# giolucasd/ssrl-vit-mae-jepa

Hardware: AMD Instinct MI355X
Metric: images/sec pretrain step (fwd+bwd+opt), ViT-S/8 96px MAE, 1/2/4/8 MI355X (higher is better)
Workload: dtype bf16; 1 GPU; ViT-S/8 96px MAE (enc 384x12x6h, dec 192x2x6h, mask_ratio 0.75), batch 2000/GPU, full step; global_batch=2000, per_gpu_batch=2000, parallelism=dp1

## Files before the change

ssrl_vit_mae_jepa_amd/csrc/engine.hip:

```cpp
#include <string>
#include <vector>
#include <cmath>
#include <cstring>
#include <cstdlib>
#include <cstdint>
#include "kernels.h"

namespace mae {

static thread_local char g_err[1024] = "";
void set_error(const char* fmt, ...) {
  va_list ap;
  va_start(ap, fmt);
  vsnprintf(g_err, sizeof(g_err), fmt, ap);
  va_end(ap);
}
int hip_fail(hipError_t err, const char* what, const char* file, int line) {
  set_error("HIP error %d (%s) at %s:%d: %s", (int)err, hipGetErrorString(err), file, line, what);
  return 2;
}

struct ParamInfo {
  std::string name;
  int64_t offset = 0, numel = 0;
// ... 21 lines not shown

using namespace mae;

struct mae_engine {
  mae_config_t cfg;
  int act = MAE_F32;
  int D, depth, H, Dd, dd, Hd, P, L, G, C, img, p, mlp;
  int PO;
  std::vector<ParamInfo> params;
  int64_t arena_elems = 0, trainable_elems = 0, trans_elems = 0;
  int i_enc_mask, i_cls, i_pos, i_patch_w, i_patch_b, i_norm_w, i_norm_b;
  int i_dec_mask, i_dec_pos, i_de_w, i_de_b, i_dn_w, i_dn_b, i_pred_w, i_pred_b;
  std::vector<BlockRefs> enc, dec;
  bool timers_on = false;
  TimerSlot timers[TK_COUNT];
  int side_mode = -1;
  hipStream_t side = nullptr;
  std::vector<hipEvent_t> ev_pool;
  size_t ev_used = 0;
  PartialsTable ln_tab;
  hipEvent_t pending[4] = {nullptr, nullptr, nullptr, nullptr};
};

namespace mae {

static int add_param(mae_engine* e, const std::string& name, std::initializer_list<int64_t> shape, int flags) {
  ParamInfo pi;
  pi.name = name;
  pi.ndim = (int)shape.size();
  pi.numel = 1;
  int i = 0;
  for (int64_t s : shape) { pi.shape[i++] = s; pi.numel *= s; }
  pi.flags = flags;
  e->params.push_back(pi);
  return (int)e->params.size() - 1;
}
// ... 18 lines not shown

struct LayerBufs {
  int64_t x_mid, ln1, mean1, rstd1, qkv, lse, att, ln2, mean2, rstd2, fc1_pre, fc1_act;
};

struct Plan {
  int B, k, m;
  int dec_B, dec_T;
  int64_t Me, Md, Mp;
  int64_t keep32, mask32, inv, pred_rows;
  int64_t patchA;
  std::vector<int64_t> enc_x, dec_x;
  std::vector<LayerBufs> enc, dec;
  int64_t enc_norm, enc_mean, enc_rstd, xdec, dec_norm, dec_mean, dec_rstd, pred;
  int64_t branch_a, branch_b;
  int64_t dpred, d_decn, dres, dres_c, d_ln, d_att, d_qkv, d_hidden, d_xdec, dtok;
  int64_t ln_partial, ln_partial_stride, split_partial, wgrad_scratch, loss_scratch;
  int64_t total;
};

static Plan make_plan_ex(const mae_engine* e, int B, int k, int dec_B, int dec_T, int m_seq) {
  Plan pl;
  pl.B = B; pl.k = k; pl.m = m_seq;
  pl.dec_B = dec_B; pl.dec_T = dec_T;
  pl.Me = (int64_t)B * k; pl.Md = (int64_t)dec_B * dec_T; pl.Mp = (int64_t)dec_B * m_seq;
  const int64_t as = (int64_t)dtype_size(e->act);
  int64_t off = 0;
  auto take = [&](int64_t bytes) { const int64_t o = off; off += round_up(std::max<int64_t>(bytes, 4), 256); return o; };
  pl.keep32 = take(pl.Me * 4);
  pl.mask32 = take(pl.Mp * 4);
  pl.inv = take(pl.Md * 4);
// ... 19 lines not shown
  };
  layers(e->depth, pl.Me, e->D, e->H, k, pl.enc_x, pl.enc);
  pl.enc_norm = take(pl.Me * e->D * as); pl.enc_mean = take(pl.Me * 4); pl.enc_rstd = take(pl.Me * 4);
  pl.xdec = take(pl.Me * e->Dd * as);
  layers(e->dd, pl.Md, e->Dd, e->Hd, dec_T, pl.dec_x, pl.dec);
  pl.dec_norm = take(std::max<int64_t>(pl.Mp, 1) * e->Dd * as);
  pl.dec_mean = take(std::max<int64_t>(pl.Mp, 1) * 4); pl.dec_rstd = take(std::max<int64_t>(pl.Mp, 1) * 4);
  pl.pred = take(std::max<int64_t>(pl.Mp, 1) * e->PO * 4);
  const int64_t R = std::max(pl.Me * e->D, pl.Md * e->Dd);
  pl.branch_a = take(R * as);
  pl.branch_b = take(R * as);
  pl.dpred = take(std::max<int64_t>(pl.Mp, 1) * e->PO * as);
  pl.d_decn = take(std::max<int64_t>(pl.Mp, 1) * e->Dd * as);
  pl.dres = take(R * 4);
  pl.dres_c = take(R * as);
  pl.d_ln = take(R * as);
  pl.d_att = take(R * as);
  pl.d_qkv = take(3 * R * as);
  pl.d_hidden = take((int64_t)e->mlp * R * as);
  pl.d_xdec = take(pl.Me * e->Dd * as);
  pl.dtok = take(pl.Me * e->D * as);
  const int maxd = std::max(e->D, e->Dd);
  pl.ln_partial_stride = (int64_t)2 * LN_BWD_MAX_BLOCKS * maxd * 4;
  pl.ln_partial = take(pl.ln_partial_stride * std::min(2 * (e->depth + e->dd) + 2, (int)PartialsTable::MAX));
  pl.split_partial = take((int64_t)512 * maxd * 4);
  int64_t wg = 0;
  auto wgs = [&](int64_t M, int N, int K) { wg = std::max(wg, linear_wgrad_scratch_bytes(M, N, K)); };
  wgs(pl.Me, 3 * e->D, e->D); wgs(pl.Me, e->mlp * e->D, e->D); wgs(pl.Me, e->D, e->mlp * e->D); wgs(pl.Me, e->D, e->D);
  wgs(pl.Md, 3 * e->Dd, e->Dd); wgs(pl.Md, e->mlp * e->Dd, e->Dd); wgs(pl.Md, e->Dd, e->mlp * e->Dd); wgs(pl.Md, e->Dd, e->Dd);
  wgs(pl.Me, e->D, e->P); wgs(pl.Me, e->Dd, e->D); wgs(std::max<int64_t>(pl.Mp, 1), e->PO, e->Dd);
// ... 22 lines not shown
    (void)hipEventRecord(t.ev[t.used].first, s);
    stop = t.ev[t.used].second;
    t.used++;
    t.flops += flops;
    t.bytes += bytes;
  }
  ~TimerScope() { if (stop) (void)hipEventRecord(stop, s); }
};

#define RUN(kind, flops, bytes, expr)                      \
  do {                                                     \
    TimerScope _ts(e, kind, (double)(flops), (double)(bytes), s); \
    MAE_TRY(expr);                                         \
  } while (0)

enum DepTag { DEP_DRESC = 0, DEP_HIDDEN = 1, DEP_QKV = 2, DEP_MISC = 3 };

static bool side_enabled(mae_engine* e) {
  if (e->side_mode < 0) {
    const char* v = getenv("MAE_WGRAD_STREAM");
    e->side_mode = (v && v[0] == '1') ? 1 : 0;
    if (e->side_mode == 1 && hipStreamCreateWithFlags(&e->side, hipStreamNonBlocking) != hipSuccess) e->side_mode = 0;
  }
  return e->side_mode == 1;
}
static hipEvent_t next_event(mae_engine* e) {
  if (e->ev_used == e->ev_pool.size()) {
    hipEvent_t ev;
    if (hipEventCreateWithFlags(&ev, hipEventDisableTiming) != hipSuccess) return nullptr;
    e->ev_pool.push_back(ev);
  }
  return e->ev_pool[e->ev_used++];
}
static int await_side(mae_engine* e, int tag, hipStream_t s) {
  if (e->pending[tag]) {
    MAE_HIP(hipStreamWaitEvent(s, e->pending[tag], 0));
    e->pending[tag] = nullptr;
  }
  return 0;
// ... 33 lines not shown
  RUN(TK_LINEAR, 2.0 * M * N * K, gemm_bytes(M, N, K, c.as, (int64_t)dtype_size(out_dt), mode), launch_linear_fwd(A, c.W(wi), M, N, K, c.act, ep, s));
  return 0;
}

static int dgrad(const Ctx& c, const void* dY, int wi, int64_t M, int N, int K, int mode, void* out, const void* aux) {
  mae_engine* e = c.e; hipStream_t s = c.s;
  Epi ep; ep.mode = mode; ep.aux = aux; ep.out = out; ep.out_dt = c.act;
  if (c.act == MAE_BF16) {
    RUN(TK_LINEAR, 2.0 * M * N * K, gemm_bytes(M, K, N, 2, 2, mode), launch_linear_fwd(dY, c.WT(wi), M, K, N, MAE_BF16, ep, s));
  } else {
    RUN(TK_LINEAR, 2.0 * M * N * K, gemm_bytes(M, K, N, 4, 4, mode), launch_linear_dgrad(dY, c.W(wi), M, N, K, MAE_F32, ep, s));
  }
  return 0;
}

static int wgrad(const Ctx& c, const Plan& pl, const void* dY, const void* A, int64_t M, int N, int K, int wi, int bi, int tag) {
  mae_engine* e = c.e;
  hipStream_t s = c.s;
  const bool side = side_enabled(e);
  if (side) {
    hipEvent_t ready = next_event(e);
    MAE_REQUIRE(ready, "wgrad: cannot create an event");
    MAE_HIP(hipEventRecord(ready, c.s));
    MAE_HIP(hipStreamWaitEvent(e->side, ready, 0));
    s = e->side;
  }
  RUN(TK_WGRAD, 2.0 * M * N * K, (double)(M * (N + K) * c.as + (int64_t)N * K * 4),
      launch_linear_wgrad(dY, A, M, N, K, c.act, c.Gp(wi), bi >= 0 ? c.Gp(bi) : nullptr, c.buf<>(pl.wgrad_scratch), s));
  if (side) {
    hipEvent_t done = next_event(e);
    MAE_REQUIRE(done, "wgrad: cannot create an event");
    MAE_HIP(hipEventRecord(done, e->side));
    e->pending[tag] = done;
  }
  return 0;
}

static int wgrad_pair(const Ctx& c, const Plan& pl, int64_t M, const void* dY0, const void* A0, int N0, int K0, int w0, int b0,
                      const void* dY1, const void* A1, int N1, int K1, int w1, int b1) {
  mae_engine* e = c.e;
  hipStream_t s = c.s;
  RUN(TK_WGRAD, 2.0 * M * ((double)N0 * K0 + (double)N1 * K1),
      (double)(M * (int64_t)(N0 + K0 + N1 + K1) * c.as + ((int64_t)N0 * K0 + (int64_t)N1 * K1) * 4),
      launch_linear_wgrad_pair(dY0, A0, N0, K0, c.Gp(w0), c.Gp(b0), dY1, A1, N1, K1, c.Gp(w1), c.Gp(b1), M, c.act, c.buf<>(pl.wgrad_scratch), s));
  return 0;
}

static int join_side(const Ctx& c) {
  mae_engine* e = c.e;
  if (e->side_mode == 1) {
    hipEvent_t done = next_event(e);
    MAE_REQUIRE(done, "cannot create an event");
    MAE_HIP(hipEventRecord(done, e->side));
    MAE_HIP(hipStreamWaitEvent(c.s, done, 0));
    for (auto& p : e->pending) p = nullptr;
  }
  return 0;
}

static int block_forward(const Ctx& c, const Plan& pl, const BlockRefs& r, const LayerBufs& b, int64_t M, int d, int heads, int Bn, int T,
                         int64_t x_prev, bool add_prev, int64_t x_in) {
  mae_engine* e = c.e; hipStream_t s = c.s;
  const int hd = d / heads, hid = e->mlp * d;
  const float eps = 1e-6f;
  if (add_prev) {
// ... 9 lines not shown
    MAE_TRY(linear(c, c.buf<>(b.ln2), r.fc1_w, r.fc1_b, M, hid, d, MAE_EPI_GELU_ACT, c.act, c.buf<>(b.fc1_act), nullptr, nullptr));
  else
    MAE_TRY(linear(c, c.buf<>(b.ln2), r.fc1_w, r.fc1_b, M, hid, d, MAE_EPI_GELU_GRAD, c.act, c.buf<>(b.fc1_pre), c.buf<>(b.fc1_act), nullptr));
  MAE_TRY(linear(c, c.buf<>(b.fc1_act), r.fc2_w, r.fc2_b, M, d, hid, MAE_EPI_NONE, c.act, c.buf<>(pl.branch_b), nullptr, nullptr));
  return 0;
}

static float* ln_slot(const Ctx& c, const Plan& pl) { return c.buf<float>(pl.ln_partial + (int64_t)(c.e->ln_tab.n % PartialsTable::MAX) * pl.ln_partial_stride); }

static int block_backward(const Ctx& c, const Plan& pl, const BlockRefs& r, const LayerBufs& b, int64_t M, int d, int heads, int Bn, int T,
                          int64_t x_in) {
  mae_engine* e = c.e; hipStream_t s = c.s;
  const int hd = d / heads, hid = e->mlp * d;
  float* dres = c.buf<float>(pl.dres);
  void* dres_c = c.buf<>(pl.dres_c);
  if (!side_enabled(e)) {
    MAE_TRY(dgrad(c, dres_c, r.fc2_w, M, d, hid, MAE_EPI_MUL, c.buf<>(pl.d_hidden), c.buf<>(b.fc1_pre)));
    MAE_TRY(wgrad_pair(c, pl, M, dres_c, c.buf<>(b.fc1_act), d, hid, r.fc2_w, r.fc2_b, c.buf<>(pl.d_hidden), c.buf<>(b.ln2), hid, d, r.fc1_w, r.fc1_b));
    MAE_TRY(dgrad(c, c.buf<>(pl.d_hidden), r.fc1_w, M, hid, d, MAE_EPI_NONE, c.buf<>(pl.d_ln), nullptr));
    RUN(TK_LN_BWD, 0, M * d * (12 + 2 * c.as), launch_layernorm_bwd(c.buf<>(pl.d_ln), c.act, c.buf<float>(b.x_mid), nullptr, c.P(r.ln2_w), c.buf<float>(b.mean2), c.buf<float>(b.rstd2), M, d, 1, dres, dres_c, c.Gp(r.ln2_w), c.Gp(r.ln2_b), ln_slot(c, pl), s, &e->ln_tab));
    MAE_TRY(dgrad(c, dres_c, r.proj_w, M, d, d, MAE_EPI_NONE, c.buf<>(pl.d_att), nullptr));
    RUN(TK_ATTN_BWD, 10.0 * Bn * heads * (double)T * T * hd, M * 9 * d * c.as, launch_attention_bwd(c.buf<>(b.qkv), c.buf<>(b.att), c.buf<>(pl.d_att), c.buf<float>(b.lse), Bn, T, heads, hd, c.act, c.buf<>(pl.d_qkv), s));
    MAE_TRY(wgrad_pair(c, pl, M, dres_c, c.buf<>(b.att), d, d, r.proj_w, r.proj_b, c.buf<>(pl.d_qkv), c.buf<>(b.ln1), 3 * d, d, r.qkv_w, r.qkv_b));
    MAE_TRY(dgrad(c, c.buf<>(pl.d_qkv), r.qkv_w, M, 3 * d, d, MAE_EPI_NONE, c.buf<>(pl.d_ln), nullptr));
    RUN(TK_LN_BWD, 0, M * d * (12 + 2 * c.as), launch_layernorm_bwd(c.buf<>(pl.d_ln), c.act, c.buf<float>(x_in), nullptr, c.P(r.ln1_w), c.buf<float>(b.mean1), c.buf<float>(b.rstd1), M, d, 1, dres, dres_c, c.Gp(r.ln1_w), c.Gp(r.ln1_b), ln_slot(c, pl), s, &e->ln_tab));
    return 0;
  }
  MAE_TRY(wgrad(c, pl, dres_c, c.buf<>(b.fc1_act), M, d, hid, r.fc2_w, r.fc2_b, DEP_DRESC));
  MAE_TRY(await_side(e, DEP_HIDDEN, s));
  MAE_TRY(dgrad(c, dres_c, r.fc2_w, M, d, hid, MAE_EPI_MUL, c.buf<>(pl.d_hidden), c.buf<>(b.fc1_pre)));
  MAE_TRY(wgrad(c, pl, c.buf<>(pl.d_hidden), c.buf<>(b.ln2), M, hid, d, r.fc1_w, r.fc1_b, DEP_HIDDEN));
  MAE_TRY(dgrad(c, c.buf<>(pl.d_hidden), r.fc1_w, M, hid, d, MAE_EPI_NONE, c.buf<>(pl.d_ln), nullptr));
  MAE_TRY(await_side(e, DEP_DRESC, s));
  RUN(TK_LN_BWD, 0, M * d * (12 + 2 * c.as), launch_layernorm_bwd(c.buf<>(pl.d_ln), c.act, c.buf<float>(b.x_mid), nullptr, c.P(r.ln2_w), c.buf<float>(b.mean2), c.buf<float>(b.rstd2), M, d, 1, dres, dres_c, c.Gp(r.ln2_w), c.Gp(r.ln2_b), ln_slot(c, pl), s, &e->ln_tab));
  MAE_TRY(wgrad(c, pl, dres_c, c.buf<>(b.att), M, d, d, r.proj_w, r.proj_b, DEP_DRESC));
  MAE_TRY(dgrad(c, dres_c, r.proj_w, M, d, d, MAE_EPI_NONE, c.buf<>(pl.d_att), nullptr));
  MAE_TRY(await_side(e, DEP_QKV, s));
  RUN(TK_ATTN_BWD, 10.0 * Bn * heads * (double)T * T * hd, M * 9 * d * c.as, launch_attention_bwd(c.buf<>(b.qkv), c.buf<>(b.att), c.buf<>(pl.d_att), c.buf<float>(b.lse), Bn, T, heads, hd, c.act, c.buf<>(pl.d_qkv), s));
  MAE_TRY(wgrad(c, pl, c.buf<>(pl.d_qkv), c.buf<>(b.ln1), M, 3 * d, d, r.qkv_w, r.qkv_b, DEP_QKV));
  MAE_TRY(dgrad(c, c.buf<>(pl.d_qkv), r.qkv_w, M, 3 * d, d, MAE_EPI_NONE, c.buf<>(pl.d_ln), nullptr));
  MAE_TRY(await_side(e, DEP_DRESC, s));
  RUN(TK_LN_BWD, 0, M * d * (12 + 2 * c.as), launch_layernorm_bwd(c.buf<>(pl.d_ln), c.act, c.buf<float>(x_in), nullptr, c.P(r.ln1_w), c.buf<float>(b.mean1), c.buf<float>(b.rstd1), M, d, 1, dres, dres_c, c.Gp(r.ln1_w), c.Gp(r.ln1_b), ln_slot(c, pl), s, &e->ln_tab));
  return 0;
}

static int check_call(const mae_engine* e, const void* params, const void* wcache, int B, int k, const void* ws, int64_t ws_bytes,
                      Plan* pl, const char* who) {
  MAE_REQUIRE(e, "%s: null engine", who);
  MAE_REQUIRE(params && ws, "%s: null params/workspace", who);
  MAE_REQUIRE(e->act == MAE_F32 || wcache, "%s: bf16 engine needs the weight cache", who);
  MAE_REQUIRE(B > 0 && k >= 1 && k <= e->L, "%s: batch %d / num_keep %d out of range (L = %d)", who, B, k, e->L);
  MAE_REQUIRE((int64_t)B * e->L * std::max(3 * e->D, e->mlp * std::max(e->D, e->Dd)) < (1ll << 40), "%s: batch too large", who);
  *pl = make_plan(e, B, k);
  MAE_REQUIRE(ws_bytes >= pl->total, "%s: workspace too small (%lld < %lld bytes)", who, (long long)ws_bytes, (long long)pl->total);
  MAE_REQUIRE(((uintptr_t)ws & 255) == 0 && ((uintptr_t)params & 15) == 0, "%s: workspace must be 256-byte aligned, params 16-byte", who);
  return 0;
// ... 49 lines not shown
  return 0;
}

static int reach_point(const Ctx& c, int j) {
  mae_engine* e = c.e; hipStream_t s = c.s;
  if (!c.ready || !c.ready[j]) return 0;
  if (e->ln_tab.n > 0) {
    RUN(TK_LN_BWD, 0, 0, launch_sum_partials_many(e->ln_tab, s));
    e->ln_tab.n = 0;
  }
  MAE_TRY(join_side(c));
  MAE_HIP(hipEventRecord((hipEvent_t)c.ready[j], s));
  return 0;
}

static void backward_begin(const Ctx& c) {
  mae_engine* e = c.e;
  e->ev_used = 0;
  for (auto& p : e->pending) p = nullptr;
  e->ln_tab.n = 0;
}
static int backward_end(const Ctx& c) {
  mae_engine* e = c.e; hipStream_t s = c.s;
  if (e->ln_tab.n > 0) RUN(TK_LN_BWD, 0, 0, launch_sum_partials_many(e->ln_tab, s));
  e->ln_tab.n = 0;
  return join_side(c);
}

static int backward_decoder_impl(const Ctx& c, const Plan& pl, const JepaSeq* jp = nullptr) {
  mae_engine* e = c.e; hipStream_t s = c.s;
  float* dres = c.buf<float>(pl.dres);
  void* dres_c = c.buf<>(pl.dres_c);
  MAE_TRY(wgrad(c, pl, c.buf<>(pl.dpred), c.buf<>(pl.dec_norm), pl.Mp, e->PO, e->Dd, e->i_pred_w, e->i_pred_b, DEP_MISC));
  MAE_TRY(dgrad(c, c.buf<>(pl.dpred), e->i_pred_w, pl.Mp, e->PO, e->Dd, MAE_EPI_NONE, c.buf<>(pl.d_decn), nullptr));
  MAE_TRY(await_side(e, DEP_DRESC, s));
// ... 15 lines not shown
  float* dres = c.buf<float>(pl.dres);
  void* dres_c = c.buf<>(pl.dres_c);
  MAE_TRY(await_side(e, DEP_DRESC, s));
  RUN(TK_LN_BWD, 0, pl.Me * e->D * (12 + 2 * c.as), launch_layernorm_bwd(c.buf<>(pl.d_ln), c.act, c.buf<float>(pl.enc_x[e->depth]), nullptr, c.P(e->i_norm_w), c.buf<float>(pl.enc_mean), c.buf<float>(pl.enc_rstd), pl.Me, e->D, 0, dres, dres_c, c.Gp(e->i_norm_w), c.Gp(e->i_norm_b), ln_slot(c, pl), s, &e->ln_tab));
  for (int i = e->depth - 1; i >= 0; --i) {
    MAE_TRY(block_backward(c, pl, e->enc[i], pl.enc[i], pl.Me, e->D, e->H, pl.B, pl.k, pl.enc_x[i]));
    if (i > 0) MAE_TRY(reach_point(c, e->depth - i));
  }
  RUN(TK_DATA, 0, pl.Me * e->D * (4 + c.as), launch_visible_grad_split(dres, c.buf<int32_t>(pl.keep32), pl.Me, e->D, c.act, c.buf<>(pl.dtok), c.Gp(e->i_cls), c.buf<float>(pl.split_partial), s));
  MAE_TRY(wgrad(c, pl, c.buf<>(pl.dtok), c.buf<>(pl.patchA), pl.Me, e->D, e->P, e->i_patch_w, e->i_patch_b, DEP_MISC));
  return 0;
}

static int backward_impl(const Ctx& c, const Plan& pl, const float* d_x_encoded_extra = nullptr, const JepaSeq* jp = nullptr) {
  mae_engine* e = c.e; hipStream_t s = c.s;
  backward_begin(c);
  MAE_TRY(backward_decoder_impl(c, pl, jp));
  if (d_x_encoded_extra) MAE_TRY(launch_add_into(d_x_encoded_extra, c.buf<>(pl.d_ln), c.act, pl.Me * e->D, s));
  MAE_TRY(backward_encoder_impl(c, pl));
  MAE_TRY(backward_end(c));
  if (c.ready && c.ready[e->depth]) MAE_HIP(hipEventRecord((hipEvent_t)c.ready[e->depth], s));
  return 0;
}

}

extern "C" const char* mae_last_error(void) { return mae::g_err; }
extern "C" int mae_abi_version(void) { return MAE_ABI_VERSION; }

extern "C" int mae_engine_create(const mae_config_t* cfg, mae_engine_t** out) {
  MAE_REQUIRE(cfg && out, "mae_engine_create: null argument");
// ... 10 lines not shown
  for (int hd : {cfg->embed_dim / cfg->num_heads, cfg->decoder_embed_dim / cfg->decoder_num_heads})
    MAE_REQUIRE(hd == 16 || hd == 24 || hd == 32 || hd == 48 || hd == 64,
                "head dim %d is not supported by the attention kernels (16, 24, 32, 48 or 64): choose num_heads accordingly", hd);
  const int P = cfg->patch_size * cfg->patch_size * cfg->in_chans;
  MAE_REQUIRE(P % 4 == 0, "patch_size^2 * in_chans must be a multiple of 4");
  MAE_REQUIRE(cfg->pred_dim >= 0 && cfg->pred_dim % 4 == 0, "pred_dim must be 0 (pixels) or a multiple of 4");
  mae_engine* e = new mae_engine();
  e->cfg = *cfg;
  e->act = cfg->act_dtype;
  e->D = cfg->embed_dim; e->depth = cfg->depth; e->H = cfg->num_heads;
  e->Dd = cfg->decoder_embed_dim; e->dd = cfg->decoder_depth; e->Hd = cfg->decoder_num_heads;
  e->C = cfg->in_chans; e->img = cfg->image_size; e->p = cfg->patch_size;
  e->G = e->img / e->p; e->L = e->G * e->G + 1; e->P = P;
  e->mlp = cfg->mlp_ratio > 0 ? cfg->mlp_ratio : 4;
  e->PO = cfg->pred_dim > 0 ? cfg->pred_dim : P;
  const int T = MAE_PARAM_TRAINABLE, M = MAE_PARAM_TRAINABLE | MAE_PARAM_MATRIX;
  e->i_enc_mask = add_param(e, "encoder.mask_token", {1, 1, e->D}, MAE_PARAM_UNUSED);
  e->i_cls = add_param(e, "encoder.vit.cls_token", {1, 1, e->D}, T);
  e->i_pos = add_param(e, "encoder.vit.pos_embed", {1, e->L, e->D}, MAE_PARAM_FROZEN);
  e->i_patch_w = add_param(e, "encoder.vit.patch_embed.proj.weight", {e->D, e->C, e->p, e->p}, M);
  e->i_patch_b = add_param(e, "encoder.vit.patch_embed.proj.bias", {e->D}, T);
  for (int i = 0; i < e->depth; ++i) e->enc.push_back(add_block(e, "encoder.vit.blocks." + std::to_string(i), e->D, e->mlp));
  e->i_norm_w = add_param(e, "encoder.vit.norm.weight", {e->D}, T);
  e->i_norm_b = add_param(e, "encoder.vit.norm.bias", {e->D}, T);
  e->i_dec_mask = add_param(e, "decoder.mask_token", {1, 1, e->Dd}, T);
  e->i_dec_pos = add_param(e, "decoder.decoder_pos_embed", {1, e->L, e->Dd}, MAE_PARAM_FROZEN);
  e->i_de_w = add_param(e, "decoder.decoder_embed.weight", {e->Dd, e->D}, M);
  e->i_de_b = add_param(e, "decoder.decoder_embed.bias", {e->Dd}, T);
  for (int i = 0; i < e->dd; ++i) e->dec.push_back(add_block(e, "decoder.decoder_blocks." + std::to_string(i), e->Dd, e->mlp));
  e->i_dn_w = add_param(e, "decoder.decoder_norm.weight", {e->Dd}, T);
// ... 121 lines not shown
  Ctx c{e, params, (const char*)wcache, grads, (char*)workspace, s, e->act, (int64_t)dtype_size(e->act)};
  MAE_TRY(launch_cast(d_pred, MAE_F32, c.buf<>(pl.dpred), e->act, pl.Mp * e->PO, s));
  return backward_impl(c, pl, d_x_encoded_extra);
}

extern "C" int mae_engine_backward_decoder(mae_engine_t* e, const float* params, const void* wcache, const float* d_pred,
                                           int32_t batch, int32_t num_keep, int32_t num_mask, void* workspace,
                                           int64_t workspace_bytes, float* grads, float* d_x_encoded, void* stream) {
  Plan pl;
  MAE_TRY(check_call(e, params, wcache, batch, num_keep, workspace, workspace_bytes, &pl, "mae_engine_backward_decoder"));
  MAE_REQUIRE(d_pred && grads, "mae_engine_backward_decoder: null d_pred/grads");
  MAE_REQUIRE(num_mask == pl.m && pl.m > 0, "mae_engine_backward_decoder: num_mask mismatch");
  hipStream_t s = (hipStream_t)stream;
  Ctx c{e, params, (const char*)wcache, grads, (char*)workspace, s, e->act, (int64_t)dtype_size(e->act)};
  MAE_TRY(launch_cast(d_pred, MAE_F32, c.buf<>(pl.dpred), e->act, pl.Mp * e->PO, s));
  backward_begin(c);
  MAE_TRY(backward_decoder_impl(c, pl));
  MAE_TRY(backward_end(c));
  if (d_x_encoded) MAE_TRY(launch_cast(c.buf<>(pl.d_ln), e->act, d_x_encoded, MAE_F32, pl.Me * e->D, s));
  return 0;
}

extern "C" int mae_engine_backward_encoder(mae_engine_t* e, const float* params, const void* wcache, const float* d_x_encoded,
                                           int32_t batch, int32_t num_keep, void* workspace, int64_t workspace_bytes,
                                           float* grads, void* stream) {
  Plan pl;
  MAE_TRY(check_call(e, params, wcache, batch, num_keep, workspace, workspace_bytes, &pl, "mae_engine_backward_encoder"));
  MAE_REQUIRE(d_x_encoded && grads, "mae_engine_backward_encoder: null d_x_encoded/grads");
  hipStream_t s = (hipStream_t)stream;
  Ctx c{e, params, (const char*)wcache, grads, (char*)workspace, s, e->act, (int64_t)dtype_size(e->act)};
  MAE_TRY(launch_cast(d_x_encoded, MAE_F32, c.buf<>(pl.d_ln), e->act, pl.Me * e->D, s));
  backward_begin(c);
  MAE_TRY(backward_encoder_impl(c, pl));
  return backward_end(c);
}

extern "C" int64_t mae_engine_encoder_grad_elems(const mae_engine_t* e) { return e ? e->params[e->i_dec_mask].offset : 0; }

extern "C" int mae_engine_decoder_decode(mae_engine_t* e, const float* params, const void* wcache, const float* x, int32_t batch,
                                         void* workspace, int64_t workspace_bytes, float* out, void* stream) {
  Plan pl;
  MAE_TRY(check_call(e, params, wcache, batch, 1, workspace, workspace_bytes, &pl, "mae_engine_decoder_decode"));
  MAE_REQUIRE(x && out, "mae_engine_decoder_decode: null x/out");
  hipStream_t s = (hipStream_t)stream;
  Ctx c{e, params, (const char*)wcache, nullptr, (char*)workspace, s, e->act, (int64_t)dtype_size(e->act)};
  MAE_TRY(launch_add_rows_pos(x, c.P(e->i_dec_pos), pl.Md, e->L, e->Dd, c.buf<float>(pl.dec_x[0]), s));
  for (int i = 0; i < e->dd; ++i)
// ... 285 lines not shown
  MAE_TRY(forward_encoder_impl(c, pl, images, image_dtype, nullptr));
  const bool cls = pool == MAE_POOL_CLS;
  void* dfeat = enc_bwd ? (cls ? c.buf<>(cp.dpooled) : c.buf<>(pl.d_ln)) : nullptr;
  RUN(TK_LOSS, 2.0 * B * C * D * (train ? 2 : 1), (cls ? (double)B * D : (double)pl.Me * D) * c.as + (double)C * D * 4 + (enc_bwd && !cls ? (double)pl.Me * D * c.as : 0.0),
      launch_classifier_head(c.buf<>(pl.enc_norm), e->act, B, L, D, pool, head, head + (int64_t)C * D, C, labels, grad_scale, logits,
                             c.buf<float>(cp.row_loss), c.buf<int32_t>(cp.row_correct), loss_out, correct_out,
                             train ? c.buf<float>(cp.pooled) : nullptr, train ? c.buf<float>(cp.dlogits) : nullptr, dfeat,
                             c.buf<float>(pl.enc_mean), c.buf<float>(pl.enc_rstd), c.buf<float>(cp.mean_c), c.buf<float>(cp.rstd_c),
                             enc_bwd && cls ? c.buf<int32_t>(cp.cls_rows) : nullptr, s));
  if (!train) return 0;
  RUN(TK_WGRAD, 2.0 * B * C * D, (double)B * (C + D) * 4, launch_classifier_head_wgrad(c.buf<float>(cp.dlogits), c.buf<float>(cp.pooled), B, C, D,
                                                                                    c.buf<float>(cp.head_partial), c.buf<float>(cp.head_sum), head_grads, s));
  if (!enc_bwd) return 0;
  float* dres = c.buf<float>(pl.dres);
  void* dres_c = c.buf<>(pl.dres_c);
  backward_begin(c);
  MAE_TRY(await_side(e, DEP_DRESC, s));
  if (cls) {
    RUN(TK_DATA, 0, (pl.Me - B) * D * (4 + c.as), launch_zero_token_rows(pl.Me, L, D, e->act, dres, dres_c, s));
    RUN(TK_LN_BWD, 0, (int64_t)B * D * (12 + 2 * c.as), launch_layernorm_bwd(c.buf<>(cp.dpooled), e->act, c.buf<float>(pl.enc_x[e->depth]), c.buf<int32_t>(cp.cls_rows), c.P(e->i_norm_w), c.buf<float>(cp.mean_c), c.buf<float>(cp.rstd_c), B, D, 0, dres, dres_c, c.Gp(e->i_norm_w), c.Gp(e->i_norm_b), ln_slot(c, pl), s, &e->ln_tab));
  } else {
    RUN(TK_LN_BWD, 0, pl.Me * D * (12 + 2 * c.as), launch_layernorm_bwd(c.buf<>(pl.d_ln), e->act, c.buf<float>(pl.enc_x[e->depth]), nullptr, c.P(e->i_norm_w), c.buf<float>(pl.enc_mean), c.buf<float>(pl.enc_rstd), pl.Me, D, 0, dres, dres_c, c.Gp(e->i_norm_w), c.Gp(e->i_norm_b), ln_slot(c, pl), s, &e->ln_tab));
  }
  for (int i = e->depth - 1; i >= e->depth - train_blocks; --i)
    MAE_TRY(block_backward(c, pl, e->enc[i], pl.enc[i], pl.Me, D, e->H, B, L, pl.enc_x[i]));
  if (train_embed) {
    RUN(TK_DATA, 0, pl.Me * D * (4 + c.as), launch_full_grad_split(dres, B, L, D, e->act, c.buf<>(pl.dtok), pos_grad, c.Gp(e->i_cls), c.buf<float>(cp.pos_partial), s));
    MAE_TRY(wgrad(c, pl, c.buf<>(pl.dtok), c.buf<>(pl.patchA), pl.Me, D, e->P, e->i_patch_w, e->i_patch_b, DEP_MISC));
  }
  return backward_end(c);
}
// ... 130 lines not shown
```

ssrl_vit_mae_jepa_amd/csrc/k_layernorm.hip:

```cpp
#include "kernels.h"

#ifndef MAE_LN_NT
#define MAE_LN_NT 5
#endif
#if MAE_LN_NT & 1
#define LN_ST_A store4_nt
#else
#define LN_ST_A store4
#endif
#if MAE_LN_NT & 2
#define LN_ST_B store4_nt
#else
#define LN_ST_B store4
#endif
#if MAE_LN_NT & 4
#define LN_LD load4_nt
#else
#define LN_LD load4
#endif

namespace mae {

template <int LPR>
__device__ __forceinline__ float group_sum(float v) {
// ... 135 lines not shown
    }
    s1 = group_sum<LPR>(s1) * inv_d;
    s2 = group_sum<LPR>(s2) * inv_d;
#pragma unroll
    for (int i = 0; i < NV; ++i) {
      const int c = li + LPR * i;
      if (c < D4 && live) {
        f32x4 d = (g[i] - s1 - xh[i] * s2) * rs;
        float* pd = dx_io + src * dim + c * 4;
        if (accumulate) d += load4(pd);
        LN_ST_A(pd, d);
        if (dx_copy) LN_ST_B(dx_copy + src * dim + c * 4, d);
      }
    }
  }
#pragma unroll
  for (int i = 0; i < NV; ++i) {
    const int c = li + LPR * i;
    if (c < D4) {
      store4(red + ((wave * RPW + sub) * 2 + 0) * dim + c * 4, dg[i]);
      store4(red + ((wave * RPW + sub) * 2 + 1) * dim + c * 4, db[i]);
    }
  }
  __syncthreads();
  for (int c = threadIdx.x; c < 2 * dim; c += 256) {
    float v = 0.f;
#pragma unroll
    for (int gidx = 0; gidx < 4 * RPW; ++gidx) v += red[gidx * 2 * dim + c];
    partial[(int64_t)blockIdx.x * 2 * dim + c] = v;
  }
}

int launch_layernorm_bwd(const void* dy, int dy_dt, const float* x, const int32_t* row_map, const float* gamma,
                         const float* mean, const float* rstd, int64_t rows, int dim, int accumulate, float* dx_io,
                         void* dx_copy, float* dgamma, float* dbeta, float* partial, hipStream_t s, PartialsTable* defer) {
  MAE_REQUIRE(dy && x && gamma && mean && rstd && dx_io && dgamma && dbeta && partial && rows > 0, "layernorm_bwd: null buffer");
  MAE_REQUIRE(dim % 4 == 0 && dim >= 4 && dim <= 1024, "layernorm: dim %d must be a multiple of 4 in [4, 1024]", dim);
  if (defer && defer->n == PartialsTable::MAX) {
    MAE_TRY(launch_sum_partials_many(*defer, s));
    defer->n = 0;
  }
  const int lpr = ln_lanes_per_row(dim / 4), nv = (int)cdiv(dim / 4, lpr);
  const int grid = (int)std::min<int64_t>(cdiv(rows, 4 * (64 / lpr)), LN_BWD_MAX_BLOCKS);
  const size_t lds = (size_t)8 * (64 / lpr) * dim * sizeof(float);
#define LNB(T, NV, LPR) hipLaunchKernelGGL((layernorm_bwd_kernel<T, NV, LPR>), dim3(grid), dim3(256), lds, s, (const T*)dy, x, row_map, gamma, mean, rstd, rows, dim, accumulate, dx_io, (T*)dx_copy, partial)
#define LNB_NV(T, LPR) switch (nv) { case 1: LNB(T, 1, LPR); break; case 2: LNB(T, 2, LPR); break; case 3: LNB(T, 3, LPR); break; default: LNB(T, 4, LPR); }
#define LNB_LPR(T) switch (lpr) { case 16: LNB_NV(T, 16) break; case 32: LNB_NV(T, 32) break; default: LNB_NV(T, 64) }
  if (dy_dt == MAE_BF16) { LNB_LPR(bf16) } else { LNB_LPR(float) }
#undef LNB_LPR
#undef LNB_NV
#undef LNB
  MAE_LAUNCH_CHECK();
  if (defer) {
    const int i = defer->n++;
    if (i == 0) defer->block_begin[0] = 0;
    defer->partial[i] = partial; defer->out0[i] = dgamma; defer->out1[i] = dbeta;
    defer->G[i] = grid; defer->C[i] = 2 * dim; defer->split[i] = dim;
    defer->block_begin[i + 1] = defer->block_begin[i] + (int)cdiv(2 * dim, 32);
    return 0;
// ... 27 lines not shown
```

ssrl_vit_mae_jepa_amd/csrc/kernels.h:

```cpp
#pragma once
#include "common.cuh"

namespace mae {

int launch_mask_from_noise(const float* noise, int B, int L, int k, int64_t* keep64, int64_t* mask64,
                           int32_t* keep32, int32_t* mask32, hipStream_t s);
int launch_idx_to_i32(const int64_t* src, int32_t* dst, int64_t n, hipStream_t s);
int launch_idx_to_i64(const int32_t* src, int64_t* dst, int64_t n, hipStream_t s);
int launch_build_inverse(const int32_t* keep32, int B, int k, int L, int32_t* inv, hipStream_t s);
int launch_build_row_map(const int32_t* idx32, int B, int n_per, int L, int32_t* rows, hipStream_t s);

int launch_gather_patches(const float* images, const int32_t* tok, int B, int k, int C, int img, int p, int dt,
                          void* out, hipStream_t s);
int launch_assemble_visible(float* x, const int32_t* tok, const float* cls, const float* pos, int64_t rows, int D,
                            hipStream_t s);
int launch_visible_grad_split(const float* dx, const int32_t* tok, int64_t rows, int D, int dt, void* dtok,
                              float* dcls, float* partial, hipStream_t s);
int launch_decoder_assemble(const void* xdec, int dt, const int32_t* inv, const float* mask_token, const float* pos,
                            int B, int k, int L, int Dd, float* out, hipStream_t s);
int launch_zero_unpredicted_rows(const int32_t* inv, int64_t rows, int Tseq, int m, int D, int act, float* dres, void* dres_c, hipStream_t s);
int launch_decoder_assemble_bwd(const float* dx, const int32_t* inv, const int32_t* keep, int B, int k, int L, int Dd,
                                int dt, void* d_xdec, float* d_mask_token, float* partial, hipStream_t s);
int launch_patchify_gather(const float* images, const int32_t* mask32, int B, int m, int C, int img, int p,
                           float* target, hipStream_t s);
// ... 70 lines not shown
int launch_layernorm_fwd(const float* x, const void* branch, float* x_out, const int32_t* row_map, const float* gamma,
                         const float* beta, float eps, int64_t rows, int dim, int y_dt, void* y, float* mean, float* rstd,
                         hipStream_t s);
struct PartialsTable {
  static constexpr int MAX = 64;
  int n = 0;
  const float* partial[MAX];
  float *out0[MAX], *out1[MAX];
  int G[MAX], C[MAX], split[MAX], block_begin[MAX + 1];
};
int launch_sum_partials_many(const PartialsTable& tab, hipStream_t s);
int launch_layernorm_bwd(const void* dy, int dy_dt, const float* x, const int32_t* row_map, const float* gamma,
                         const float* mean, const float* rstd, int64_t rows, int dim, int accumulate, float* dx_io,
                         void* dx_copy, float* dgamma, float* dbeta, float* partial, hipStream_t s, PartialsTable* defer = nullptr);
constexpr int LN_BWD_MAX_BLOCKS = 1024;

int num_cus();

struct Epi {
  int mode = MAE_EPI_NONE;
  const float* bias = nullptr;
  const void* aux = nullptr;
  void* out = nullptr;
  void* out2 = nullptr;
  int out_dt = MAE_F32;
};
int launch_linear_fwd(const void* A, const void* W, int64_t M, int N, int K, int dt, const Epi& epi, hipStream_t s);
int launch_linear_dgrad(const void* dY, const void* W, int64_t M, int N, int K, int dt, const Epi& epi, hipStream_t s);
int64_t linear_wgrad_scratch_bytes(int64_t M, int N, int K);
int launch_linear_wgrad(const void* dY, const void* A, int64_t M, int N, int K, int dt, float* dW, float* db,
// ... 11 lines not shown
```

Baseline: 91590 images/s.

## Halve LayerNorm-backward LDS via two-pass reduction and rework side-stream wgrad pairing

The LayerNorm backward kernel now reduces dgamma/dbeta partials in two column passes, halving its dynamic LDS allocation so more blocks can be resident per CU, at the cost of an extra barrier. Separately, the optional side-stream weight-gradient path (MAE_WGRAD_STREAM=1) now issues paired wgrads on the side stream, double-buffers the residual gradient copy, and is disabled during graph capture. The stream change is off by default, so the default path gains only the LDS change.

```diff
diff --git a/ssrl_vit_mae_jepa_amd/csrc/engine.hip b/ssrl_vit_mae_jepa_amd/csrc/engine.hip
--- a/ssrl_vit_mae_jepa_amd/csrc/engine.hip
+++ b/ssrl_vit_mae_jepa_amd/csrc/engine.hip
@@ -59,12 +59,13 @@
   std::vector<BlockRefs> enc, dec;
   bool timers_on = false;
   TimerSlot timers[TK_COUNT];
-  int side_mode = -1;
+  int side_mode = 0;
+  bool side_active = false;
   hipStream_t side = nullptr;
   std::vector<hipEvent_t> ev_pool;
   size_t ev_used = 0;
   PartialsTable ln_tab;
-  hipEvent_t pending[4] = {nullptr, nullptr, nullptr, nullptr};
+  hipEvent_t pending[5] = {nullptr, nullptr, nullptr, nullptr, nullptr};
 };
 
 namespace mae {
@@ -113,7 +114,7 @@
   std::vector<LayerBufs> enc, dec;
   int64_t enc_norm, enc_mean, enc_rstd, xdec, dec_norm, dec_mean, dec_rstd, pred;
   int64_t branch_a, branch_b;
-  int64_t dpred, d_decn, dres, dres_c, d_ln, d_att, d_qkv, d_hidden, d_xdec, dtok;
+  int64_t dpred, d_decn, dres, dres_c, dres_c2, d_ln, d_att, d_qkv, d_hidden, d_xdec, dtok;
   int64_t ln_partial, ln_partial_stride, split_partial, wgrad_scratch, loss_scratch;
   int64_t total;
 };
@@ -163,6 +164,7 @@
   pl.d_decn = take(std::max<int64_t>(pl.Mp, 1) * e->Dd * as);
   pl.dres = take(R * 4);
   pl.dres_c = take(R * as);
+  pl.dres_c2 = take(R * as);
   pl.d_ln = take(R * as);
   pl.d_att = take(R * as);
   pl.d_qkv = take(3 * R * as);
@@ -215,15 +217,17 @@
     MAE_TRY(expr);                                         \
   } while (0)
 
-enum DepTag { DEP_DRESC = 0, DEP_HIDDEN = 1, DEP_QKV = 2, DEP_MISC = 3 };
-
-static bool side_enabled(mae_engine* e) {
-  if (e->side_mode < 0) {
-    const char* v = getenv("MAE_WGRAD_STREAM");
-    e->side_mode = (v && v[0] == '1') ? 1 : 0;
-    if (e->side_mode == 1 && hipStreamCreateWithFlags(&e->side, hipStreamNonBlocking) != hipSuccess) e->side_mode = 0;
-  }
-  return e->side_mode == 1;
+enum DepTag { DEP_DRESC = 0, DEP_DRESC2 = 1, DEP_HIDDEN = 2, DEP_QKV = 3, DEP_MISC = 4 };
+
+static int side_begin(mae_engine* e, hipStream_t s) {
+  e->side_active = false;
+  if (e->side_mode != 1) return 0;
+  hipStreamCaptureStatus st = hipStreamCaptureStatusNone;
+  MAE_HIP(hipStreamIsCapturing(s, &st));
+  if (st != hipStreamCaptureStatusNone) return 0;
+  if (!e->side) MAE_HIP(hipStreamCreateWithFlags(&e->side, hipStreamNonBlocking));
+  e->side_active = true;
+  return 0;
 }
 static hipEvent_t next_event(mae_engine* e) {
   if (e->ev_used == e->ev_pool.size()) {
@@ -287,41 +291,51 @@
   return 0;
 }
 
+static int fork_side(const Ctx& c, hipStream_t* s) {
+  mae_engine* e = c.e;
+  hipEvent_t ready = next_event(e);
+  MAE_REQUIRE(ready, "wgrad: cannot create an event");
+  MAE_HIP(hipEventRecord(ready, c.s));
+  MAE_HIP(hipStreamWaitEvent(e->side, ready, 0));
+  *s = e->side;
+  return 0;
+}
+static int mark_side(mae_engine* e, int a, int b) {
+  hipEvent_t done = next_event(e);
+  MAE_REQUIRE(done, "wgrad: cannot create an event");
+  MAE_HIP(hipEventRecord(done, e->side));
+  e->pending[a] = done;
+  e->pending[b] = done;
+  return 0;
+}
+
 static int wgrad(const Ctx& c, const Plan& pl, const void* dY, const void* A, int64_t M, int N, int K, int wi, int bi, int tag) {
   mae_engine* e = c.e;
   hipStream_t s = c.s;
-  const bool side = side_enabled(e);
-  if (side) {
-    hipEvent_t ready = next_event(e);
-    MAE_REQUIRE(ready, "wgrad: cannot create an event");
-    MAE_HIP(hipEventRecord(ready, c.s));
-    MAE_HIP(hipStreamWaitEvent(e->side, ready, 0));
-    s = e->side;
-  }
+  const bool side = e->side_active;
+  if (side) MAE_TRY(fork_side(c, &s));
   RUN(TK_WGRAD, 2.0 * M * N * K, (double)(M * (N + K) * c.as + (int64_t)N * K * 4),
       launch_linear_wgrad(dY, A, M, N, K, c.act, c.Gp(wi), bi >= 0 ? c.Gp(bi) : nullptr, c.buf<>(pl.wgrad_scratch), s));
-  if (side) {
-    hipEvent_t done = next_event(e);
-    MAE_REQUIRE(done, "wgrad: cannot create an event");
-    MAE_HIP(hipEventRecord(done, e->side));
-    e->pending[tag] = done;
-  }
+  if (side) MAE_TRY(mark_side(e, tag, tag));
   return 0;
 }
 
 static int wgrad_pair(const Ctx& c, const Plan& pl, int64_t M, const void* dY0, const void* A0, int N0, int K0, int w0, int b0,
-                      const void* dY1, const void* A1, int N1, int K1, int w1, int b1) {
+                      const void* dY1, const void* A1, int N1, int K1, int w1, int b1, int tag0, int tag1) {
   mae_engine* e = c.e;
   hipStream_t s = c.s;
+  const bool side = e->side_active;
+  if (side) MAE_TRY(fork_side(c, &s));
   RUN(TK_WGRAD, 2.0 * M * ((double)N0 * K0 + (double)N1 * K1),
       (double)(M * (int64_t)(N0 + K0 + N1 + K1) * c.as + ((int64_t)N0 * K0 + (int64_t)N1 * K1) * 4),
       launch_linear_wgrad_pair(dY0, A0, N0, K0, c.Gp(w0), c.Gp(b0), dY1, A1, N1, K1, c.Gp(w1), c.Gp(b1), M, c.act, c.buf<>(pl.wgrad_scratch), s));
+  if (side) MAE_TRY(mark_side(e, tag0, tag1));
   return 0;
 }
 
 static int join_side(const Ctx& c) {
   mae_engine* e = c.e;
-  if (e->side_mode == 1) {
+  if (e->side_active) {
     hipEvent_t done = next_event(e);
     MAE_REQUIRE(done, "cannot create an event");
     MAE_HIP(hipEventRecord(done, e->side));
@@ -361,32 +375,27 @@
   const int hd = d / heads, hid = e->mlp * d;
   float* dres = c.buf<float>(pl.dres);
   void* dres_c = c.buf<>(pl.dres_c);
-  if (!side_enabled(e)) {
-    MAE_TRY(dgrad(c, dres_c, r.fc2_w, M, d, hid, MAE_EPI_MUL, c.buf<>(pl.d_hidden), c.buf<>(b.fc1_pre)));
-    MAE_TRY(wgrad_pair(c, pl, M, dres_c, c.buf<>(b.fc1_act), d, hid, r.fc2_w, r.fc2_b, c.buf<>(pl.d_hidden), c.buf<>(b.ln2), hid, d, r.fc1_w, r.fc1_b));
-    MAE_TRY(dgrad(c, c.buf<>(pl.d_hidden), r.fc1_w, M, hid, d, MAE_EPI_NONE, c.buf<>(pl.d_ln), nullptr));
-    RUN(TK_LN_BWD, 0, M * d * (12 + 2 * c.as), launch_layernorm_bwd(c.buf<>(pl.d_ln), c.act, c.buf<float>(b.x_mid), nullptr, c.P(r.ln2_w), c.buf<float>(b.mean2), c.buf<float>(b.rstd2), M, d, 1, dres, dres_c, c.Gp(r.ln2_w), c.Gp(r.ln2_b), ln_slot(c, pl), s, &e->ln_tab));
-    MAE_TRY(dgrad(c, dres_c, r.proj_w, M, d, d, MAE_EPI_NONE, c.buf<>(pl.d_att), nullptr));
-    RUN(TK_ATTN_BWD, 10.0 * Bn * heads * (double)T * T * hd, M * 9 * d * c.as, launch_attention_bwd(c.buf<>(b.qkv), c.buf<>(b.att), c.buf<>(pl.d_att), c.buf<float>(b.lse), Bn, T, heads, hd, c.act, c.buf<>(pl.d_qkv), s));
-    MAE_TRY(wgrad_pair(c, pl, M, dres_c, c.buf<>(b.att), d, d, r.proj_w, r.proj_b, c.buf<>(pl.d_qkv), c.buf<>(b.ln1), 3 * d, d, r.qkv_w, r.qkv_b));
-    MAE_TRY(dgrad(c, c.buf<>(pl.d_qkv), r.qkv_w, M, 3 * d, d, MAE_EPI_NONE, c.buf<>(pl.d_ln), nullptr));
-    RUN(TK_LN_BWD, 0, M * d * (12 + 2 * c.as), launch_layernorm_bwd(c.buf<>(pl.d_ln), c.act, c.buf<float>(x_in), nullptr, c.P(r.ln1_w), c.buf<float>(b.mean1), c.buf<float>(b.rstd1), M, d, 1, dres, dres_c, c.Gp(r.ln1_w), c.Gp(r.ln1_b), ln_slot(c, pl), s, &e->ln_tab));
-    return 0;
-  }
-  MAE_TRY(wgrad(c, pl, dres_c, c.buf<>(b.fc1_act), M, d, hid, r.fc2_w, r.fc2_b, DEP_DRESC));
+  void* dres_m = e->side_active ? c.buf<>(pl.dres_c2) : dres_c;
   MAE_TRY(await_side(e, DEP_HIDDEN, s));
   MAE_TRY(dgrad(c, dres_c, r.fc2_w, M, d, hid, MAE_EPI_MUL, c.buf<>(pl.d_hidden), c.buf<>(b.fc1_pre)));
-  MAE_TRY(wgrad(c, pl, c.buf<>(pl.d_hidden), c.buf<>(b.ln2), M, hid, d, r.fc1_w, r.fc1_b, DEP_HIDDEN));
+  if (!e->side_active)
+    MAE_TRY(wgrad_pair(c, pl, M, dres_c, c.buf<>(b.fc1_act), d, hid, r.fc2_w, r.fc2_b, c.buf<>(pl.d_hidden), c.buf<>(b.ln2), hid, d, r.fc1_w, r.fc1_b, DEP_DRESC, DEP_HIDDEN));
   MAE_TRY(dgrad(c, c.buf<>(pl.d_hidden), r.fc1_w, M, hid, d, MAE_EPI_NONE, c.buf<>(pl.d_ln), nullptr));
-  MAE_TRY(await_side(e, DEP_DRESC, s));
-  RUN(TK_LN_BWD, 0, M * d * (12 + 2 * c.as), launch_layernorm_bwd(c.buf<>(pl.d_ln), c.act, c.buf<float>(b.x_mid), nullptr, c.P(r.ln2_w), c.buf<float>(b.mean2), c.buf<float>(b.rstd2), M, d, 1, dres, dres_c, c.Gp(r.ln2_w), c.Gp(r.ln2_b), ln_slot(c, pl), s, &e->ln_tab));
-  MAE_TRY(wgrad(c, pl, dres_c, c.buf<>(b.att), M, d, d, r.proj_w, r.proj_b, DEP_DRESC));
-  MAE_TRY(dgrad(c, dres_c, r.proj_w, M, d, d, MAE_EPI_NONE, c.buf<>(pl.d_att), nullptr));
+  if (e->side_active) {
+    MAE_TRY(wgrad_pair(c, pl, M, dres_c, c.buf<>(b.fc1_act), d, hid, r.fc2_w, r.fc2_b, c.buf<>(pl.d_hidden), c.buf<>(b.ln2), hid, d, r.fc1_w, r.fc1_b, DEP_DRESC, DEP_HIDDEN));
+    MAE_TRY(await_side(e, DEP_DRESC2, s));
+  }
+  RUN(TK_LN_BWD, 0, M * d * (12 + 2 * c.as), launch_layernorm_bwd(c.buf<>(pl.d_ln), c.act, c.buf<float>(b.x_mid), nullptr, c.P(r.ln2_w), c.buf<float>(b.mean2), c.buf<float>(b.rstd2), M, d, 1, dres, dres_m, c.Gp(r.ln2_w), c.Gp(r.ln2_b), ln_slot(c, pl), s, &e->ln_tab));
+  MAE_TRY(dgrad(c, dres_m, r.proj_w, M, d, d, MAE_EPI_NONE, c.buf<>(pl.d_att), nullptr));
   MAE_TRY(await_side(e, DEP_QKV, s));
   RUN(TK_ATTN_BWD, 10.0 * Bn * heads * (double)T * T * hd, M * 9 * d * c.as, launch_attention_bwd(c.buf<>(b.qkv), c.buf<>(b.att), c.buf<>(pl.d_att), c.buf<float>(b.lse), Bn, T, heads, hd, c.act, c.buf<>(pl.d_qkv), s));
-  MAE_TRY(wgrad(c, pl, c.buf<>(pl.d_qkv), c.buf<>(b.ln1), M, 3 * d, d, r.qkv_w, r.qkv_b, DEP_QKV));
+  if (!e->side_active)
+    MAE_TRY(wgrad_pair(c, pl, M, dres_m, c.buf<>(b.att), d, d, r.proj_w, r.proj_b, c.buf<>(pl.d_qkv), c.buf<>(b.ln1), 3 * d, d, r.qkv_w, r.qkv_b, DEP_DRESC, DEP_QKV));
   MAE_TRY(dgrad(c, c.buf<>(pl.d_qkv), r.qkv_w, M, 3 * d, d, MAE_EPI_NONE, c.buf<>(pl.d_ln), nullptr));
-  MAE_TRY(await_side(e, DEP_DRESC, s));
+  if (e->side_active) {
+    MAE_TRY(wgrad_pair(c, pl, M, dres_m, c.buf<>(b.att), d, d, r.proj_w, r.proj_b, c.buf<>(pl.d_qkv), c.buf<>(b.ln1), 3 * d, d, r.qkv_w, r.qkv_b, DEP_DRESC2, DEP_QKV));
+    MAE_TRY(await_side(e, DEP_DRESC, s));
+  }
   RUN(TK_LN_BWD, 0, M * d * (12 + 2 * c.as), launch_layernorm_bwd(c.buf<>(pl.d_ln), c.act, c.buf<float>(x_in), nullptr, c.P(r.ln1_w), c.buf<float>(b.mean1), c.buf<float>(b.rstd1), M, d, 1, dres, dres_c, c.Gp(r.ln1_w), c.Gp(r.ln1_b), ln_slot(c, pl), s, &e->ln_tab));
   return 0;
 }
@@ -466,11 +475,13 @@
   return 0;
 }
 
-static void backward_begin(const Ctx& c) {
+static int backward_begin(const Ctx& c) {
   mae_engine* e = c.e;
+  MAE_TRY(side_begin(e, c.s));
   e->ev_used = 0;
   for (auto& p : e->pending) p = nullptr;
   e->ln_tab.n = 0;
+  return 0;
 }
 static int backward_end(const Ctx& c) {
   mae_engine* e = c.e; hipStream_t s = c.s;
@@ -516,7 +527,7 @@
 
 static int backward_impl(const Ctx& c, const Plan& pl, const float* d_x_encoded_extra = nullptr, const JepaSeq* jp = nullptr) {
   mae_engine* e = c.e; hipStream_t s = c.s;
-  backward_begin(c);
+  MAE_TRY(backward_begin(c));
   MAE_TRY(backward_decoder_impl(c, pl, jp));
   if (d_x_encoded_extra) MAE_TRY(launch_add_into(d_x_encoded_extra, c.buf<>(pl.d_ln), c.act, pl.Me * e->D, s));
   MAE_TRY(backward_encoder_impl(c, pl));
@@ -557,6 +568,8 @@
   e->G = e->img / e->p; e->L = e->G * e->G + 1; e->P = P;
   e->mlp = cfg->mlp_ratio > 0 ? cfg->mlp_ratio : 4;
   e->PO = cfg->pred_dim > 0 ? cfg->pred_dim : P;
+  const char* ws = getenv("MAE_WGRAD_STREAM");
+  e->side_mode = (ws && ws[0] == '1') ? 1 : 0;
   const int T = MAE_PARAM_TRAINABLE, M = MAE_PARAM_TRAINABLE | MAE_PARAM_MATRIX;
   e->i_enc_mask = add_param(e, "encoder.mask_token", {1, 1, e->D}, MAE_PARAM_UNUSED);
   e->i_cls = add_param(e, "encoder.vit.cls_token", {1, 1, e->D}, T);
@@ -708,7 +721,7 @@
   hipStream_t s = (hipStream_t)stream;
   Ctx c{e, params, (const char*)wcache, grads, (char*)workspace, s, e->act, (int64_t)dtype_size(e->act)};
   MAE_TRY(launch_cast(d_pred, MAE_F32, c.buf<>(pl.dpred), e->act, pl.Mp * e->PO, s));
-  backward_begin(c);
+  MAE_TRY(backward_begin(c));
   MAE_TRY(backward_decoder_impl(c, pl));
   MAE_TRY(backward_end(c));
   if (d_x_encoded) MAE_TRY(launch_cast(c.buf<>(pl.d_ln), e->act, d_x_encoded, MAE_F32, pl.Me * e->D, s));
@@ -724,7 +737,7 @@
   hipStream_t s = (hipStream_t)stream;
   Ctx c{e, params, (const char*)wcache, grads, (char*)workspace, s, e->act, (int64_t)dtype_size(e->act)};
   MAE_TRY(launch_cast(d_x_encoded, MAE_F32, c.buf<>(pl.d_ln), e->act, pl.Me * e->D, s));
-  backward_begin(c);
+  MAE_TRY(backward_begin(c));
   MAE_TRY(backward_encoder_impl(c, pl));
   return backward_end(c);
 }
@@ -1040,7 +1053,7 @@
   if (!enc_bwd) return 0;
   float* dres = c.buf<float>(pl.dres);
   void* dres_c = c.buf<>(pl.dres_c);
-  backward_begin(c);
+  MAE_TRY(backward_begin(c));
   MAE_TRY(await_side(e, DEP_DRESC, s));
   if (cls) {
     RUN(TK_DATA, 0, (pl.Me - B) * D * (4 + c.as), launch_zero_token_rows(pl.Me, L, D, e->act, dres, dres_c, s));
diff --git a/ssrl_vit_mae_jepa_amd/csrc/k_layernorm.hip b/ssrl_vit_mae_jepa_amd/csrc/k_layernorm.hip
--- a/ssrl_vit_mae_jepa_amd/csrc/k_layernorm.hip
+++ b/ssrl_vit_mae_jepa_amd/csrc/k_layernorm.hip
@@ -173,20 +173,29 @@
       }
     }
   }
-#pragma unroll
-  for (int i = 0; i < NV; ++i) {
-    const int c = li + LPR * i;
-    if (c < D4) {
-      store4(red + ((wave * RPW + sub) * 2 + 0) * dim + c * 4, dg[i]);
-      store4(red + ((wave * RPW + sub) * 2 + 1) * dim + c * 4, db[i]);
-    }
-  }
-  __syncthreads();
-  for (int c = threadIdx.x; c < 2 * dim; c += 256) {
-    float v = 0.f;
-#pragma unroll
-    for (int gidx = 0; gidx < 4 * RPW; ++gidx) v += red[gidx * 2 * dim + c];
-    partial[(int64_t)blockIdx.x * 2 * dim + c] = v;
+  const int S4 = (D4 + LN_BWD_LDS_PASSES - 1) / LN_BWD_LDS_PASSES, W = S4 * 4;
+  for (int p = 0; p < LN_BWD_LDS_PASSES; ++p) {
+    const int lo4 = p * S4, hi4 = min(lo4 + S4, D4);
+#pragma unroll
+    for (int i = 0; i < NV; ++i) {
+      const int c = li + LPR * i;
+      if (c >= lo4 && c < hi4) {
+        store4(red + ((wave * RPW + sub) * 2 + 0) * W + (c - lo4) * 4, dg[i]);
+        store4(red + ((wave * RPW + sub) * 2 + 1) * W + (c - lo4) * 4, db[i]);
+      }
+    }
+    __syncthreads();
+    const int w = (hi4 - lo4) * 4;
+    for (int idx = threadIdx.x; idx < 2 * W; idx += 256) {
+      const int which = idx >= W, col = idx - which * W;
+      if (col < w) {
+        float v = 0.f;
+#pragma unroll
+        for (int gidx = 0; gidx < 4 * RPW; ++gidx) v += red[(gidx * 2 + which) * W + col];
+        partial[(int64_t)blockIdx.x * 2 * dim + which * dim + lo4 * 4 + col] = v;
+      }
+    }
+    __syncthreads();
   }
 }
 
@@ -201,7 +210,7 @@
   }
   const int lpr = ln_lanes_per_row(dim / 4), nv = (int)cdiv(dim / 4, lpr);
   const int grid = (int)std::min<int64_t>(cdiv(rows, 4 * (64 / lpr)), LN_BWD_MAX_BLOCKS);
-  const size_t lds = (size_t)8 * (64 / lpr) * dim * sizeof(float);
+  const size_t lds = (size_t)8 * (64 / lpr) * 4 * cdiv(dim / 4, LN_BWD_LDS_PASSES) * sizeof(float);
 #define LNB(T, NV, LPR) hipLaunchKernelGGL((layernorm_bwd_kernel<T, NV, LPR>), dim3(grid), dim3(256), lds, s, (const T*)dy, x, row_map, gamma, mean, rstd, rows, dim, accumulate, dx_io, (T*)dx_copy, partial)
 #define LNB_NV(T, LPR) switch (nv) { case 1: LNB(T, 1, LPR); break; case 2: LNB(T, 2, LPR); break; case 3: LNB(T, 3, LPR); break; default: LNB(T, 4, LPR); }
 #define LNB_LPR(T) switch (lpr) { case 16: LNB_NV(T, 16) break; case 32: LNB_NV(T, 32) break; default: LNB_NV(T, 64) }
diff --git a/ssrl_vit_mae_jepa_amd/csrc/kernels.h b/ssrl_vit_mae_jepa_amd/csrc/kernels.h
--- a/ssrl_vit_mae_jepa_amd/csrc/kernels.h
+++ b/ssrl_vit_mae_jepa_amd/csrc/kernels.h
@@ -108,6 +108,7 @@
                          const float* mean, const float* rstd, int64_t rows, int dim, int accumulate, float* dx_io,
                          void* dx_copy, float* dgamma, float* dbeta, float* partial, hipStream_t s, PartialsTable* defer = nullptr);
 constexpr int LN_BWD_MAX_BLOCKS = 1024;
+constexpr int LN_BWD_LDS_PASSES = 2;
 
 int num_cus();
 
```

Measured after the change: 91510 images/s. Within noise of the previous version (-0.1%).
